# faris-k/self-supervised-wafermaps

Hardware: AMD Instinct MI355X
Metric: imgs/sec (SimCLR ResNet18, bs=256, 224^2) (higher is better)
Workload: dtype bf16; 1 GPU; SimCLR ResNet-18, 256 wafers/GPU/step, two 3x224x224 views, NT-Xent in-batch negatives, SGD (BASELINE.json configs[1]); per_gpu_batch=256, global_batch=256, parallelism=dp1, hip_graph=True, backward_stage_graphs=1, parallel_branches=two views through the backbone

## Files before the change

self-supervised-wafermaps_amd/csrc/pool.hip:

```cpp
#include "common.h"

namespace {

constexpr int PL_THREADS = 256;

__device__ __forceinline__ void up8(const uint4 v, float (&f)[8]) {
  f[0] = bf2f((uint16_t)(v.x & 0xffff)); f[1] = bf2f((uint16_t)(v.x >> 16));
  f[2] = bf2f((uint16_t)(v.y & 0xffff)); f[3] = bf2f((uint16_t)(v.y >> 16));
  f[4] = bf2f((uint16_t)(v.z & 0xffff)); f[5] = bf2f((uint16_t)(v.z >> 16));
  f[6] = bf2f((uint16_t)(v.w & 0xffff)); f[7] = bf2f((uint16_t)(v.w >> 16));
}

__global__ __launch_bounds__(PL_THREADS) void maxpool_fwd(const uint16_t* __restrict__ x, int N, int H,
                                                          int W, int C, int P, int Q,
                                                          uint16_t* __restrict__ y,
                                                          uint8_t* __restrict__ idx) {
  const int cpr = C >> 3;
  const long long total = (long long)N * P * Q * cpr;
  for (long long t = (long long)blockIdx.x * PL_THREADS + threadIdx.x; t < total;
       t += (long long)gridDim.x * PL_THREADS) {
    const int c0 = (int)(t % cpr) * 8;
    long long pix = t / cpr;
    const int q = (int)(pix % Q);
    pix /= Q;
    const int p = (int)(pix % P), n = (int)(pix / P);
    float best[8];
    int bi[8];
#pragma unroll
    for (int e = 0; e < 8; ++e) {
      best[e] = -INFINITY;
      bi[e] = 0;
    }
    bool first = true;
#pragma unroll
    for (int kh = 0; kh < 3; ++kh)
#pragma unroll
      for (int kw = 0; kw < 3; ++kw) {
        const int h = p * 2 - 1 + kh, w = q * 2 - 1 + kw;
        if ((unsigned)h < (unsigned)H && (unsigned)w < (unsigned)W) {
          float f[8];
          up8(*reinterpret_cast<const uint4*>(x + ((size_t)(n * H + h) * W + w) * C + c0), f);
#pragma unroll
          for (int e = 0; e < 8; ++e)
            if (first || f[e] > best[e]) {
              best[e] = f[e];
              bi[e] = kh * 3 + kw;
            }
          first = false;
        }
      }
    const size_t o = ((size_t)(n * P + p) * Q + q) * C + c0;
    *reinterpret_cast<uint4*>(y + o) = make_uint4(pack_bf2(best[0], best[1]), pack_bf2(best[2], best[3]),
                                                  pack_bf2(best[4], best[5]), pack_bf2(best[6], best[7]));
    uint2 pk;
    pk.x = bi[0] | (bi[1] << 8) | (bi[2] << 16) | (bi[3] << 24);
    pk.y = bi[4] | (bi[5] << 8) | (bi[6] << 16) | (bi[7] << 24);
    *reinterpret_cast<uint2*>(idx + o) = pk;
  }
}

__global__ __launch_bounds__(PL_THREADS) void bn_relu_maxpool_fwd(const uint16_t* __restrict__ x,
                                                                  const float* __restrict__ scale,
                                                                  const float* __restrict__ shift, int N,
                                                                  int H, int W, int C, int P, int Q,
                                                                  int imgs_per_group,
                                                                  uint16_t* __restrict__ y,
                                                                  uint8_t* __restrict__ idx,
                                                                  uint16_t* __restrict__ xsel, const WmDiv d_cpr,
                                                                  const WmDiv d_q, const WmDiv d_p, const WmDiv d_ipg) {
  const uint32_t cpr = (uint32_t)C >> 3;
  const uint32_t total = (uint32_t)N * P * Q * cpr;
  for (uint32_t t = blockIdx.x * PL_THREADS + threadIdx.x; t < total; t += gridDim.x * PL_THREADS) {
    uint32_t rc, rq, rp;
    uint32_t pix = wm_divmod(t, d_cpr, rc);
    const int c0 = (int)rc * 8;
    pix = wm_divmod(pix, d_q, rq);
    const int n = (int)wm_divmod(pix, d_p, rp);
    const int q = (int)rq, p = (int)rp;
    const int g = (int)wm_div((uint32_t)n, d_ipg);
    float sc[8], sh[8], bx[8];
#pragma unroll
    for (int e = 0; e < 8; ++e) {
      sc[e] = scale[(size_t)g * C + c0 + e];
      sh[e] = shift[(size_t)g * C + c0 + e];
    }
    float best[8];
    int bi[8];
#pragma unroll
    for (int e = 0; e < 8; ++e) {
      best[e] = -INFINITY;
      bi[e] = 0;
    }
    bool first = true;
#pragma unroll
    for (int kh = 0; kh < 3; ++kh)
#pragma unroll
      for (int kw = 0; kw < 3; ++kw) {
        const int h = p * 2 - 1 + kh, w = q * 2 - 1 + kw;
        if ((unsigned)h < (unsigned)H && (unsigned)w < (unsigned)W) {
          float f[8];
          up8(*reinterpret_cast<const uint4*>(x + ((size_t)(n * H + h) * W + w) * C + c0), f);
#pragma unroll
          for (int e = 0; e < 8; ++e) {
            const float v = bf2f(f2bf(fmaxf(fmaf(f[e], sc[e], sh[e]), 0.f)));
            if (first || v > best[e]) {
              best[e] = v;
              bi[e] = kh * 3 + kw;
              bx[e] = f[e];
            }
          }
          first = false;
        }
      }
    const size_t o = ((size_t)(n * P + p) * Q + q) * C + c0;
    *reinterpret_cast<uint4*>(y + o) = make_uint4(pack_bf2(best[0], best[1]), pack_bf2(best[2], best[3]),
                                                  pack_bf2(best[4], best[5]), pack_bf2(best[6], best[7]));
    uint2 pk;
    pk.x = bi[0] | (bi[1] << 8) | (bi[2] << 16) | (bi[3] << 24);
    pk.y = bi[4] | (bi[5] << 8) | (bi[6] << 16) | (bi[7] << 24);
    *reinterpret_cast<uint2*>(idx + o) = pk;
    if (xsel != nullptr)
      *reinterpret_cast<uint4*>(xsel + o) = make_uint4(pack_bf2(bx[0], bx[1]), pack_bf2(bx[2], bx[3]),
                                                       pack_bf2(bx[4], bx[5]), pack_bf2(bx[6], bx[7]));
  }
}

__global__ __launch_bounds__(PL_THREADS) void maxpool_bwd(const uint16_t* __restrict__ dy,
                                                          const uint8_t* __restrict__ idx, int N, int H,
                                                          int W, int C, int P, int Q,
                                                          uint16_t* __restrict__ dx) {
  const int cpr = C >> 3;
  const long long total = (long long)N * H * W * cpr;
  for (long long t = (long long)blockIdx.x * PL_THREADS + threadIdx.x; t < total;
       t += (long long)gridDim.x * PL_THREADS) {
    const int c0 = (int)(t % cpr) * 8;
    long long pix = t / cpr;
    const int w = (int)(pix % W);
    pix /= W;
    const int h = (int)(pix % H), n = (int)(pix / H);
    float g[8];
#pragma unroll
    for (int e = 0; e < 8; ++e) g[e] = 0.f;
    const int p_lo = h >> 1, p_hi = (h + 1) >> 1, q_lo = w >> 1, q_hi = (w + 1) >> 1;
    for (int p = p_lo; p <= p_hi; ++p) {
      if (p >= P) continue;
      const int kh = h - (2 * p - 1);
      for (int q = q_lo; q <= q_hi; ++q) {
        if (q >= Q) continue;
        const int code = kh * 3 + (w - (2 * q - 1));
        const size_t o = ((size_t)(n * P + p) * Q + q) * C + c0;
        const uint2 pk = *reinterpret_cast<const uint2*>(idx + o);
        float d[8];
        up8(*reinterpret_cast<const uint4*>(dy + o), d);
#pragma unroll
        for (int e = 0; e < 8; ++e) {
          const int ie = (int)(((e < 4 ? pk.x : pk.y) >> (8 * (e & 3))) & 0xff);
          g[e] += ie == code ? d[e] : 0.f;
        }
      }
    }
    *reinterpret_cast<uint4*>(dx + ((size_t)(n * H + h) * W + w) * C + c0) =
        make_uint4(pack_bf2(g[0], g[1]), pack_bf2(g[2], g[3]), pack_bf2(g[4], g[5]), pack_bf2(g[6], g[7]));
  }
}

__global__ __launch_bounds__(PL_THREADS) void gap_fwd(const uint16_t* __restrict__ x, int N, int HW, int C,
                                                      uint16_t* __restrict__ y) {
  const int cpr = C >> 3;
  const int t = blockIdx.x * PL_THREADS + threadIdx.x;
  if (t >= N * cpr) return;
  const int n = t / cpr, c0 = (t - n * cpr) * 8;
  float s[8];
#pragma unroll
  for (int e = 0; e < 8; ++e) s[e] = 0.f;
  for (int i = 0; i < HW; ++i) {
    float f[8];
    up8(*reinterpret_cast<const uint4*>(x + ((size_t)n * HW + i) * C + c0), f);
#pragma unroll
    for (int e = 0; e < 8; ++e) s[e] += f[e];
  }
  const float inv = 1.0f / (float)HW;
  *reinterpret_cast<uint4*>(y + (size_t)n * C + c0) =
      make_uint4(pack_bf2(s[0] * inv, s[1] * inv), pack_bf2(s[2] * inv, s[3] * inv),
                 pack_bf2(s[4] * inv, s[5] * inv), pack_bf2(s[6] * inv, s[7] * inv));
}

__global__ __launch_bounds__(PL_THREADS) void gap_bwd(const uint16_t* __restrict__ dy, int N, int HW, int C,
                                                      uint16_t* __restrict__ dx) {
  const int cpr = C >> 3;
  const long long total = (long long)N * HW * cpr;
  const float inv = 1.0f / (float)HW;
  for (long long t = (long long)blockIdx.x * PL_THREADS + threadIdx.x; t < total;
       t += (long long)gridDim.x * PL_THREADS) {
    const int c0 = (int)(t % cpr) * 8;
    const long long pix = t / cpr;
    const int n = (int)(pix / HW);
    float d[8];
    up8(*reinterpret_cast<const uint4*>(dy + (size_t)n * C + c0), d);
    *reinterpret_cast<uint4*>(dx + (size_t)pix * C + c0) =
        make_uint4(pack_bf2(d[0] * inv, d[1] * inv), pack_bf2(d[2] * inv, d[3] * inv),
                   pack_bf2(d[4] * inv, d[5] * inv), pack_bf2(d[6] * inv, d[7] * inv));
  }
}

inline int grid_for(long long items) {
  long long b = (items + PL_THREADS - 1) / PL_THREADS;
  if (b > 4096) b = 4096;
  return b < 1 ? 1 : (int)b;
}

}

extern "C" int wm_maxpool3x3s2_fwd(const void* x, int N, int H, int W, int C, void* y, void* idx, void* stream) {
  WM_REQUIRE(x && y && idx, WM_EINVAL);
  WM_REQUIRE(N > 0 && H > 1 && W > 1 && C > 0, WM_EINVAL);
  WM_REQUIRE(C % 8 == 0, WM_EUNSUPPORTED);
  const int P = (H + 2 - 3) / 2 + 1, Q = (W + 2 - 3) / 2 + 1;
  maxpool_fwd<<<grid_for((long long)N * P * Q * (C >> 3)), PL_THREADS, 0, static_cast<hipStream_t>(stream)>>>(
      static_cast<const uint16_t*>(x), N, H, W, C, P, Q, static_cast<uint16_t*>(y), static_cast<uint8_t*>(idx));
  WM_LAUNCH_CHECK();
  return WM_OK;
}

extern "C" int wm_bn_relu_maxpool3x3s2_fwd(const void* x, const float* scale, const float* shift, int N, int H,
                                           int W, int C, int G, void* y, void* idx, void* xsel, void* stream) {
  WM_REQUIRE(x && scale && shift && y && idx, WM_EINVAL);
  WM_REQUIRE(N > 0 && H > 1 && W > 1 && C > 0 && G > 0, WM_EINVAL);
  WM_REQUIRE(C % 8 == 0 && N % G == 0, WM_EUNSUPPORTED);
  WM_REQUIRE((long long)N * H * W * (C / 8) < (1ll << 31), WM_EUNSUPPORTED);
  const int P = (H + 2 - 3) / 2 + 1, Q = (W + 2 - 3) / 2 + 1;
  bn_relu_maxpool_fwd<<<grid_for((long long)N * P * Q * (C >> 3)), PL_THREADS, 0, static_cast<hipStream_t>(stream)>>>(
      static_cast<const uint16_t*>(x), scale, shift, N, H, W, C, P, Q, N / G, static_cast<uint16_t*>(y),
      static_cast<uint8_t*>(idx), static_cast<uint16_t*>(xsel), wm_div_make((uint32_t)(C >> 3)), wm_div_make((uint32_t)Q),
      wm_div_make((uint32_t)P), wm_div_make((uint32_t)(N / G)));
  WM_LAUNCH_CHECK();
  return WM_OK;
}

extern "C" int wm_maxpool3x3s2_bwd(const void* dy, const void* idx, int N, int H, int W, int C, void* dx,
                                   void* stream) {
  WM_REQUIRE(dy && idx && dx, WM_EINVAL);
  WM_REQUIRE(N > 0 && H > 1 && W > 1 && C > 0, WM_EINVAL);
  WM_REQUIRE(C % 8 == 0, WM_EUNSUPPORTED);
  const int P = (H + 2 - 3) / 2 + 1, Q = (W + 2 - 3) / 2 + 1;
  maxpool_bwd<<<grid_for((long long)N * H * W * (C >> 3)), PL_THREADS, 0, static_cast<hipStream_t>(stream)>>>(
      static_cast<const uint16_t*>(dy), static_cast<const uint8_t*>(idx), N, H, W, C, P, Q,
      static_cast<uint16_t*>(dx));
  WM_LAUNCH_CHECK();
  return WM_OK;
}

extern "C" int wm_gap_fwd(const void* x, int N, int HW, int C, void* y, void* stream) {
  WM_REQUIRE(x && y, WM_EINVAL);
  WM_REQUIRE(N > 0 && HW > 0 && C > 0, WM_EINVAL);
  WM_REQUIRE(C % 8 == 0, WM_EUNSUPPORTED);
  gap_fwd<<<wm_cdiv((long long)N * (C >> 3), PL_THREADS), PL_THREADS, 0, static_cast<hipStream_t>(stream)>>>(
      static_cast<const uint16_t*>(x), N, HW, C, static_cast<uint16_t*>(y));
  WM_LAUNCH_CHECK();
  return WM_OK;
}

extern "C" int wm_gap_bwd(const void* dy, int N, int HW, int C, void* dx, void* stream) {
  WM_REQUIRE(dy && dx, WM_EINVAL);
  WM_REQUIRE(N > 0 && HW > 0 && C > 0, WM_EINVAL);
  WM_REQUIRE(C % 8 == 0, WM_EUNSUPPORTED);
  gap_bwd<<<grid_for((long long)N * HW * (C >> 3)), PL_THREADS, 0, static_cast<hipStream_t>(stream)>>>(
      static_cast<const uint16_t*>(dy), N, HW, C, static_cast<uint16_t*>(dx));
  WM_LAUNCH_CHECK();
  return WM_OK;
}
```

Baseline: 25180 imgs/sec.

## Process fused BN-ReLU-maxpool in vertical strips reusing shared boundary rows

Each thread now computes four consecutive output rows of the fused BN+ReLU+3x3/s2 maxpool. The row winner of the shared boundary input row is carried over instead of being reloaded and recomputed, which cuts redundant global loads and BN math. The kernel is templated on whether the pre-activation select output is needed. The bf16 rounding now uses a packed convert instruction, and the winner code and raw input bits are packed into one word. This reduces the thread count and parallelism in exchange for more work per thread, and it relies on edge-clamped loads and tie-breaking matching the old semantics.

```diff
diff --git a/self-supervised-wafermaps_amd/csrc/pool.hip b/self-supervised-wafermaps_amd/csrc/pool.hip
--- a/self-supervised-wafermaps_amd/csrc/pool.hip
+++ b/self-supervised-wafermaps_amd/csrc/pool.hip
@@ -59,69 +59,116 @@
   }
 }
 
+constexpr int PL_STRIP = 4;
+
+template <bool XSEL>
+__device__ __forceinline__ void pool_row_winner(const uint16_t* __restrict__ row, int q, int W, int C,
+                                                const float (&sc)[8], const float (&sh)[8], uint32_t code0,
+                                                float (&v)[8], uint32_t (&xc)[8]) {
+  const int wc = 2 * q;
+  const bool left = q > 0, right = wc + 1 < W;
+  const uint4 r0 = *reinterpret_cast<const uint4*>(row + (size_t)(left ? wc - 1 : wc) * C);
+  const uint4 r1 = *reinterpret_cast<const uint4*>(row + (size_t)wc * C);
+  const uint4 r2 = *reinterpret_cast<const uint4*>(row + (size_t)(right ? wc + 1 : wc) * C);
+  const uint32_t raw[3][4] = {{r0.x, r0.y, r0.z, r0.w}, {r1.x, r1.y, r1.z, r1.w}, {r2.x, r2.y, r2.z, r2.w}};
+  const uint32_t code[3] = {left ? code0 : code0 + 1, code0 + 1, code0 + 2};
+#pragma unroll
+  for (int kw = 0; kw < 3; ++kw)
+#pragma unroll
+    for (int j = 0; j < 4; ++j) {
+      const uint32_t w32 = raw[kw][j];
+      const uint32_t xb[2] = {w32 << 16, w32 & 0xffff0000u};
+      uint32_t pk;
+      asm("v_cvt_pk_bf16_f32 %0, %1, %2"
+          : "=v"(pk)
+          : "v"(fmaxf(fmaf(__builtin_bit_cast(float, xb[0]), sc[2 * j], sh[2 * j]), 0.f)),
+            "v"(fmaxf(fmaf(__builtin_bit_cast(float, xb[1]), sc[2 * j + 1], sh[2 * j + 1]), 0.f)));
+      const float t[2] = {__builtin_bit_cast(float, pk << 16), __builtin_bit_cast(float, pk & 0xffff0000u)};
+#pragma unroll
+      for (int k = 0; k < 2; ++k) {
+        const int e = 2 * j + k;
+        if (kw == 0 || t[k] > v[e]) {
+          v[e] = t[k];
+          xc[e] = XSEL ? (xb[k] | code[kw]) : code[kw];
+        }
+      }
+    }
+}
+
+template <bool XSEL>
 __global__ __launch_bounds__(PL_THREADS) void bn_relu_maxpool_fwd(const uint16_t* __restrict__ x,
                                                                   const float* __restrict__ scale,
                                                                   const float* __restrict__ shift, int N,
-                                                                  int H, int W, int C, int P, int Q,
-                                                                  int imgs_per_group,
+                                                                  int H, int W, int C, int P, int Q, int S,
                                                                   uint16_t* __restrict__ y,
                                                                   uint8_t* __restrict__ idx,
                                                                   uint16_t* __restrict__ xsel, const WmDiv d_cpr,
-                                                                  const WmDiv d_q, const WmDiv d_p, const WmDiv d_ipg) {
+                                                                  const WmDiv d_q, const WmDiv d_s, const WmDiv d_ipg) {
   const uint32_t cpr = (uint32_t)C >> 3;
-  const uint32_t total = (uint32_t)N * P * Q * cpr;
+  const uint32_t total = (uint32_t)N * S * Q * cpr;
   for (uint32_t t = blockIdx.x * PL_THREADS + threadIdx.x; t < total; t += gridDim.x * PL_THREADS) {
-    uint32_t rc, rq, rp;
+    uint32_t rc, rq, rs;
     uint32_t pix = wm_divmod(t, d_cpr, rc);
     const int c0 = (int)rc * 8;
     pix = wm_divmod(pix, d_q, rq);
-    const int n = (int)wm_divmod(pix, d_p, rp);
-    const int q = (int)rq, p = (int)rp;
+    const int n = (int)wm_divmod(pix, d_s, rs);
+    const int q = (int)rq, p0 = (int)rs * PL_STRIP;
+    const int p1 = p0 + PL_STRIP < P ? p0 + PL_STRIP : P;
     const int g = (int)wm_div((uint32_t)n, d_ipg);
-    float sc[8], sh[8], bx[8];
+    float sc[8], sh[8];
 #pragma unroll
     for (int e = 0; e < 8; ++e) {
       sc[e] = scale[(size_t)g * C + c0 + e];
       sh[e] = shift[(size_t)g * C + c0 + e];
     }
-    float best[8];
-    int bi[8];
-#pragma unroll
-    for (int e = 0; e < 8; ++e) {
-      best[e] = -INFINITY;
-      bi[e] = 0;
-    }
-    bool first = true;
-#pragma unroll
-    for (int kh = 0; kh < 3; ++kh)
-#pragma unroll
-      for (int kw = 0; kw < 3; ++kw) {
-        const int h = p * 2 - 1 + kh, w = q * 2 - 1 + kw;
-        if ((unsigned)h < (unsigned)H && (unsigned)w < (unsigned)W) {
-          float f[8];
-          up8(*reinterpret_cast<const uint4*>(x + ((size_t)(n * H + h) * W + w) * C + c0), f);
-#pragma unroll
-          for (int e = 0; e < 8; ++e) {
-            const float v = bf2f(f2bf(fmaxf(fmaf(f[e], sc[e], sh[e]), 0.f)));
-            if (first || v > best[e]) {
-              best[e] = v;
-              bi[e] = kh * 3 + kw;
-              bx[e] = f[e];
-            }
-          }
-          first = false;
-        }
-      }
-    const size_t o = ((size_t)(n * P + p) * Q + q) * C + c0;
-    *reinterpret_cast<uint4*>(y + o) = make_uint4(pack_bf2(best[0], best[1]), pack_bf2(best[2], best[3]),
-                                                  pack_bf2(best[4], best[5]), pack_bf2(best[6], best[7]));
-    uint2 pk;
-    pk.x = bi[0] | (bi[1] << 8) | (bi[2] << 16) | (bi[3] << 24);
-    pk.y = bi[4] | (bi[5] << 8) | (bi[6] << 16) | (bi[7] << 24);
-    *reinterpret_cast<uint2*>(idx + o) = pk;
-    if (xsel != nullptr)
-      *reinterpret_cast<uint4*>(xsel + o) = make_uint4(pack_bf2(bx[0], bx[1]), pack_bf2(bx[2], bx[3]),
-                                                       pack_bf2(bx[4], bx[5]), pack_bf2(bx[6], bx[7]));
+    const uint16_t* img = x + (size_t)n * H * W * C + c0;
+    const size_t rstride = (size_t)W * C;
+    float pv[8];
+    uint32_t pxc[8];
+    if (p0 > 0) {
+      pool_row_winner<XSEL>(img + (size_t)(2 * p0 - 1) * rstride, q, W, C, sc, sh, 0u, pv, pxc);
+    } else {
+#pragma unroll
+      for (int e = 0; e < 8; ++e) {
+        pv[e] = -INFINITY;
+        pxc[e] = 0u;
+      }
+    }
+    for (int p = p0; p < p1; ++p) {
+      float av[8], bv[8];
+      uint32_t axc[8], bxc[8];
+      const int hb = 2 * p + 1 < H ? 2 * p + 1 : 2 * p;
+      pool_row_winner<XSEL>(img + (size_t)(2 * p) * rstride, q, W, C, sc, sh, 3u, av, axc);
+      pool_row_winner<XSEL>(img + (size_t)hb * rstride, q, W, C, sc, sh, 6u, bv, bxc);
+      float best[8];
+      uint32_t bxcode[8];
+#pragma unroll
+      for (int e = 0; e < 8; ++e) {
+        best[e] = pv[e];
+        bxcode[e] = pxc[e];
+        if (av[e] > best[e]) {
+          best[e] = av[e];
+          bxcode[e] = axc[e];
+        }
+        if (bv[e] > best[e]) {
+          best[e] = bv[e];
+          bxcode[e] = bxc[e];
+        }
+        pv[e] = bv[e];
+        pxc[e] = bxc[e] - 6u;
+      }
+      const size_t o = ((size_t)(n * P + p) * Q + q) * C + c0;
+      *reinterpret_cast<uint4*>(y + o) = make_uint4(pack_bf2(best[0], best[1]), pack_bf2(best[2], best[3]),
+                                                    pack_bf2(best[4], best[5]), pack_bf2(best[6], best[7]));
+      uint2 pk;
+      pk.x = (bxcode[0] & 0xff) | ((bxcode[1] & 0xff) << 8) | ((bxcode[2] & 0xff) << 16) | (bxcode[3] << 24);
+      pk.y = (bxcode[4] & 0xff) | ((bxcode[5] & 0xff) << 8) | ((bxcode[6] & 0xff) << 16) | (bxcode[7] << 24);
+      *reinterpret_cast<uint2*>(idx + o) = pk;
+      if (XSEL)
+        *reinterpret_cast<uint4*>(xsel + o) =
+            make_uint4((bxcode[0] >> 16) | (bxcode[1] & 0xffff0000u), (bxcode[2] >> 16) | (bxcode[3] & 0xffff0000u),
+                       (bxcode[4] >> 16) | (bxcode[5] & 0xffff0000u), (bxcode[6] >> 16) | (bxcode[7] & 0xffff0000u));
+    }
   }
 }
 
@@ -229,10 +276,13 @@
   WM_REQUIRE(C % 8 == 0 && N % G == 0, WM_EUNSUPPORTED);
   WM_REQUIRE((long long)N * H * W * (C / 8) < (1ll << 31), WM_EUNSUPPORTED);
   const int P = (H + 2 - 3) / 2 + 1, Q = (W + 2 - 3) / 2 + 1;
-  bn_relu_maxpool_fwd<<<grid_for((long long)N * P * Q * (C >> 3)), PL_THREADS, 0, static_cast<hipStream_t>(stream)>>>(
-      static_cast<const uint16_t*>(x), scale, shift, N, H, W, C, P, Q, N / G, static_cast<uint16_t*>(y),
+  const int S = (P + PL_STRIP - 1) / PL_STRIP;
+  const int grid = grid_for((long long)N * S * Q * (C >> 3));
+  auto* kern = xsel ? bn_relu_maxpool_fwd<true> : bn_relu_maxpool_fwd<false>;
+  kern<<<grid, PL_THREADS, 0, static_cast<hipStream_t>(stream)>>>(
+      static_cast<const uint16_t*>(x), scale, shift, N, H, W, C, P, Q, S, static_cast<uint16_t*>(y),
       static_cast<uint8_t*>(idx), static_cast<uint16_t*>(xsel), wm_div_make((uint32_t)(C >> 3)), wm_div_make((uint32_t)Q),
-      wm_div_make((uint32_t)P), wm_div_make((uint32_t)(N / G)));
+      wm_div_make((uint32_t)S), wm_div_make((uint32_t)(N / G)));
   WM_LAUNCH_CHECK();
   return WM_OK;
 }
```

Measured after the change: 25230 imgs/sec (median of 5 runs). No clear change (+0.2%).
